# li-kunyi/CUT3R-SLAM

Measured on AMD Instinct MI355X. Metric: frames/sec (ViT pointmap + covisibility-graph tracking step) on 640x480, higher is better.
Workload: dtype f16

## Files before the change

### cut3r_slam_amd/_lib.py

```python
from __future__ import annotations

import ctypes as C
import os

_HERE = os.path.dirname(os.path.abspath(__file__))
LIB_PATH = os.path.join(_HERE, "libcut3r_hip.so")

c_void_p, c_int, c_float, c_ll = C.c_void_p, C.c_int, C.c_float, C.c_longlong


class GemmDesc(C.Structure):
    _fields_ = [
        ("A", c_void_p), ("B", c_void_p), ("C", c_void_p), ("bias", c_void_p), ("res1", c_void_p), ("res2", c_void_p),
        ("M", c_int), ("N", c_int), ("K", c_int), ("lda", c_int), ("ldb", c_int), ("ldc", c_int), ("ldr1", c_int),
        ("ldr2", c_int),
        ("act", c_int), ("out_f16", c_int), ("res1_f16", c_int), ("res2_f16", c_int),
        ("batch", c_int),
        ("strideA", c_ll), ("strideB", c_ll), ("strideC", c_ll), ("strideBias", c_ll), ("strideR1", c_ll),
        ("strideR2", c_ll),
        ("conv_k", c_int), ("H", c_int), ("W", c_int), ("Cin", c_int), ("conv_stride", c_int), ("Ho", c_int),
        ("Wo", c_int), ("relu_in", c_int),
        ("shuf", c_int), ("shuf_cout", c_int), ("shuf_Hin", c_int), ("shuf_Win", c_int),
        ("tile", c_int), ("stages", c_int),
        ("rope_pos", c_void_p), ("rope_table", c_void_p), ("rope_cols", c_int), ("rope_pmin", c_int), ("rope_npos", c_int),
# ... 21 lines not shown
    "cut3r_layernorm_tokens": [c_void_p, c_int, c_void_p, c_void_p, c_float, c_int, c_int, c_int, c_void_p, c_ll, c_void_p, c_ll, c_void_p,
                               c_ll, c_void_p, c_ll, c_void_p],
    "cut3r_gemm_f16": [C.POINTER(GemmDesc), c_void_p],
    "cut3r_gemm_tile_for": [C.POINTER(GemmDesc)],
    "cut3r_gemm_f16_pair": [C.POINTER(GemmDesc), C.POINTER(GemmDesc), c_void_p],
    "cut3r_gemm_kernel_for": [C.POINTER(GemmDesc)],
    "cut3r_gemm_pair_kernel_for": [C.POINTER(GemmDesc), C.POINTER(GemmDesc)],
    "cut3r_gemm_kernel_count": [],
    "cut3r_rope2d_table": [c_void_p, c_int, c_int, c_int, c_float, c_float, c_void_p],
    "cut3r_gemv_f16w": [c_void_p, c_int, c_void_p, c_int, c_void_p, c_void_p, c_int, c_int, c_int, c_int, c_int,
                        c_void_p, c_int, c_int, c_void_p],
    "cut3r_attention_variant": [c_int],
    "cut3r_attention_kernel_for": [c_int, c_int, c_int, c_int],
    "cut3r_attention_f16": [c_void_p, c_void_p, c_void_p, c_void_p, c_int, c_int, c_int, c_int, c_int,
                            c_ll, c_ll, c_ll, c_ll, c_ll, c_ll, c_ll, c_ll, c_float, c_void_p],
    "cut3r_attention_one_key_f16": [c_void_p, c_void_p, c_int, c_int, c_int, c_int, c_ll, c_ll, c_ll, c_ll, c_void_p],
    "cut3r_im2col_patch": [c_void_p, c_int, c_int, c_int, c_int, c_int, c_int, c_void_p, c_void_p],
    "cut3r_cast_f32_f16": [c_void_p, c_int, c_void_p, c_int, c_int, c_int, c_void_p],
    "cut3r_colmean": [c_void_p, c_int, c_int, c_int, c_void_p, c_void_p],
    "cut3r_colmean_batched": [c_void_p, c_int, c_ll, c_int, c_int, c_int, c_void_p, c_ll, c_void_p],
    "cut3r_upsample2x_nhwc": [c_void_p, c_void_p, c_int, c_int, c_int, c_int, c_void_p],
    "cut3r_dpt_final": [c_void_p, c_int, c_int, c_void_p, c_void_p, c_int, c_void_p, c_void_p, c_void_p],
    "cut3r_conv3x3_dpt_final": [C.POINTER(GemmDesc), c_void_p, c_void_p, c_int, c_void_p, c_ll, c_void_p, c_ll, c_void_p],
    "cut3r_postprocess_pts": [c_void_p, c_int, c_int, c_int, c_void_p, c_void_p, c_void_p],
    "cut3r_postprocess_pose": [c_void_p, c_int, c_void_p, c_void_p],
    "cut3r_patch_overlap": [c_void_p, c_void_p, c_int, c_int, c_float, c_void_p, c_void_p, c_void_p],
    "cut3r_patch_overlap_chain": [c_void_p, c_void_p, c_int, c_int, c_int, c_float, C.c_double, c_void_p, c_void_p, c_void_p, c_void_p,
                                  c_void_p, c_void_p],
    "cut3r_overlap_fwd": [c_void_p, c_int, C.POINTER(c_float), c_float, c_void_p, c_int, c_float, c_float, c_float, c_float,
                          c_int, c_int, c_int, c_void_p, c_void_p],
# ... 181 lines not shown
```

### cut3r_slam_amd/csrc/attention.hip

```cpp
#include <atomic>
#include <cmath>
#include <cstdlib>
#include <type_traits>
#include "common.h"
#include "../../include/cut3r_hip.h"

namespace {

typedef __fp16 fp16x4_t __attribute__((ext_vector_type(4)));

DEVINL void halves(float x, float& lo, float& hi) {
    const auto r = __builtin_amdgcn_permlane32_swap(__float_as_uint(x), __float_as_uint(x), false, false);
    lo = __uint_as_float(r[0]);
    hi = __uint_as_float(r[1]);
}

struct AttnArgs {
    const h16* q; const h16* k; const h16* v; h16* o;
    int Nq, Nk;
    long long q_sb, q_sn, k_sb, k_sn, v_sb, v_sn, o_sb, o_sn;
    float scale_log2;
};

template <int D, int NW>
// ... 217 lines not shown
DEVINL unsigned lds_addr(const void* p) {
    return (unsigned)(unsigned long long)(__attribute__((address_space(3))) const void*)p;
}

template <int N>
DEVINL void wait_vm() { asm volatile("s_waitcnt vmcnt(%0)" ::"n"(N) : "memory"); }
template <int P, int MAXT>
DEVINL void wait_tiles_ahead(int tiles_ahead) {
    if constexpr (MAXT == 0) wait_vm<0>();
    else {
        if (tiles_ahead >= MAXT) wait_vm<P * MAXT>();
        else wait_tiles_ahead<P, MAXT - 1>(tiles_ahead);
    }
}

template <int D, int QB, int NST, int NW>
__global__ __launch_bounds__(64 * NW, (QB == 1 ? 2 : 1)) void attn_pipe_kernel(const AttnArgs a, const int nblk, const int HB, const int H) {
    constexpr int KT = 64;
    constexpr int PPW = 8 / NW;
    constexpr int AHEAD = NST - 4;
    constexpr int DQ = D / 16;
    constexpr int DP = (D + 31) / 32;
    constexpr int CH = D / 8;
    constexpr int VOFF = KT * 128;
    constexpr int STAGE = 2 * KT * 128;
    static_assert(D % 16 == 0 && D <= 64 && NST >= 4 && (NW == 4 || NW == 8), "head dims 16..64; the ring holds tiles j-1 .. j+2 and NST-4 more in flight");
    __shared__ __attribute__((aligned(1024))) unsigned char smem[NST * STAGE];

    const int tid = threadIdx.x, lane = tid & 63;
    const int wave = __builtin_amdgcn_readfirstlane(tid >> 6);
    const int r = lane & 31, hh = lane >> 5;
    const int L = blockIdx.x;
    const int xb = (L >> 3) % nblk;
    const int bh = ((L >> 3) / nblk) * 8 + (L & 7);
    if (bh >= HB) return;
    const int h = bh % H, b = bh / H;
    const int q0 = xb * (32 * NW * QB) + wave * (32 * QB);
    const h16* qp = a.q + (size_t)b * a.q_sb + (size_t)h * D;
    const h16* kp = a.k + (size_t)b * a.k_sb + (size_t)h * D;
    const h16* vp = a.v + (size_t)b * a.v_sb + (size_t)h * D;
    const bool active = q0 < a.Nq;
    const int extra = (a.Nk > KT && (a.Nk % KT) == 1) ? 1 : 0;
    const int ntiles = (a.Nk - extra + KT - 1) / KT;

    if (CH < 8) {
        for (int i = tid; i < NST * STAGE / 16; i += 64 * NW) *reinterpret_cast<f32x4*>(smem + i * 16) = f32x4{0.f, 0.f, 0.f, 0.f};
        asm volatile("s_waitcnt lgkmcnt(0)" ::: "memory");
        asm volatile("s_barrier" ::: "memory");
    }

    auto lane_src = [&](int c, int row_limit, unsigned& ko, unsigned& vo, bool& kval, bool& vval) {
        const int row = (wave * PPW + c) * 8 + (lane >> 3), slot = lane & 7;
        const int kc = slot ^ ((row >> 1) & 7), vc = slot ^ (((row >> 1) & 1) << 2);
        const int rr = min(row, row_limit);
        ko = (unsigned)rr * (unsigned)(a.k_sn * 2) + kc * 16;
        vo = (unsigned)rr * (unsigned)(a.v_sn * 2) + vc * 16;
        kval = kc < CH;
        vval = vc < CH;
    };
// ... 32 lines not shown
            asm volatile("s_barrier" ::: "memory");
            issue(j + NST - 2);
        }
        asm volatile("s_waitcnt vmcnt(0)" ::: "memory");
        return;
    }

    half8_t qf[QB][DQ];
    f32x16 ot[QB][DP];
    float m_run[QB], l_run[QB];
#pragma unroll
    for (int qb = 0; qb < QB; qb++) {
        int qr = q0 + qb * 32 + r;
        if (qr > a.Nq - 1) qr = a.Nq - 1;
        const h16* qrow = qp + (size_t)qr * a.q_sn;
#pragma unroll
        for (int s = 0; s < DQ; s++) qf[qb][s] = *reinterpret_cast<const half8_t*>(qrow + 16 * s + 8 * hh);
#pragma unroll
        for (int d = 0; d < DP; d++)
#pragma unroll
            for (int i = 0; i < 16; i++) ot[qb][d][i] = 0.f;
        m_run[qb] = -INFINITY;
        l_run[qb] = 0.f;
        if (extra) {
            float dot = 0.f;
#pragma unroll
            for (int s = 0; s < DQ; s++) {
                const half8_t k0 = *reinterpret_cast<const half8_t*>(kp + 16 * s + 8 * hh);
#pragma unroll
                for (int j = 0; j < 8; j++) dot = fmaf((float)qf[qb][s][j], (float)k0[j], dot);
            }
            { float d0, d1; halves(dot, d0, d1); dot = d0 + d1; }
// ... 159 lines not shown
            if (__any(gflag)) {
#pragma unroll
                for (int qb = 0; qb < QB; qb++)
#pragma unroll
                    for (int d = 0; d < DP; d++)
#pragma unroll
                        for (int i = 0; i < 16; i++) ot[qb][d][i] *= alpha[qb];
            }
        }
    };
    using T0 = std::integral_constant<int, 0>;
    using T1 = std::integral_constant<int, 1>;
    using Y = std::true_type;
    using N = std::false_type;

#pragma unroll
    for (int t = 0; t < NST - 3; t++) issue(t);
    {
        wait_tiles_ahead<2 * PPW, AHEAD>(ntiles - 1);
        asm volatile("s_barrier" ::: "memory");
        issue(NST - 3);
        {
            half8_t kf[2][DQ];
#pragma unroll
            for (int kt2 = 0; kt2 < 2; kt2++)
#pragma unroll
                for (int s = 0; s < DQ; s++) kf[kt2][s] = *reinterpret_cast<const half8_t*>(smem + kt2 * 32 * 128 + koff[s]);
#pragma unroll
            for (int kt2 = 0; kt2 < 2; kt2++)
#pragma unroll
                for (int qb = 0; qb < QB; qb++) {
#pragma unroll
// ... 46 lines not shown
        }
    }
}

std::atomic<int> g_attn_variant{[] { const char* e = getenv("CUT3R_ATTN_PIPE"); return e ? atoi(e) : 1; }()};

int attn_instance(int B, int H, int Nq, int D) {
    static const long long nw4_min = [] { const char* e = getenv("CUT3R_ATTN_NW4_MIN"); return e ? atoll(e) : 384LL; }();
    if (D != 16 && D != 32 && D != 48 && D != 64 && D != 128) return 0;
    if ((D == 48 || D == 64) && g_attn_variant.load(std::memory_order_relaxed) != 0) return 104;
    const long long blocks128 = (long long)B * H * ((Nq + 127) / 128);
    return (blocks128 >= nw4_min || D >= 128) ? 4 : 2;
}

template <int D>
int launch_attn(const AttnArgs& a, int B, int H, hipStream_t s) {
    const int inst = attn_instance(B, H, a.Nq, D);
    if constexpr (D == 48 || D == 64) {
        if (inst == 104) {
            const int nblk = (a.Nq + 127) / 128, HB = H * B;
            dim3 grid((unsigned)(((HB + 7) / 8) * 8 * nblk));
            hipLaunchKernelGGL((attn_pipe_kernel<D, 1, 4, 4>), grid, dim3(256), 0, s, a, nblk, HB, H);
            return cut3r_check_launch();
        }
    }
    if (inst == 4) {
        dim3 grid((a.Nq + 127) / 128, H, B);
        hipLaunchKernelGGL((attn_kernel<D, 4>), grid, dim3(256), 0, s, a);
    } else if (inst == 2) {
        dim3 grid((a.Nq + 63) / 64, H, B);
        hipLaunchKernelGGL((attn_kernel<D, 2>), grid, dim3(128), 0, s, a);
    } else {
        return CUT3R_ERR_ARG;
    }
    return cut3r_check_launch();
}

__global__ __launch_bounds__(256) void attn_one_key_kernel(const h16* __restrict__ v, h16* __restrict__ o, int Nq, int hd8, long long v_sb,
                                                           long long o_sb, long long o_sn, long long total) {
    const long long i = (long long)blockIdx.x * 256 + threadIdx.x;
// ... 20 lines not shown
    hipLaunchKernelGGL(attn_one_key_kernel, dim3((unsigned)((total + 255) / 256)), dim3(256), 0, (hipStream_t)stream, (const h16*)v,
                       (h16*)out, Nq, (int)(hd / 8), v_sb, o_sb, o_sn, total);
    return cut3r_check_launch();
}

extern "C" int cut3r_attention_variant(int v) {
    if (v < 0) return g_attn_variant.load(std::memory_order_relaxed);
    return g_attn_variant.exchange(v ? 1 : 0, std::memory_order_relaxed);
}

extern "C" int cut3r_attention_kernel_for(int B, int H, int Nq, int D) {
    if (B <= 0 || H <= 0 || Nq <= 0) return 0;
    return attn_instance(B, H, Nq, D);
}

extern "C" int cut3r_attention_f16(const void* q, const void* k, const void* v, void* out, int B, int H, int Nq, int Nk, int D,
                                   long long q_sb, long long q_sn, long long k_sb, long long k_sn, long long v_sb, long long v_sn,
                                   long long o_sb, long long o_sn, float scale, void* stream) {
    if (!q || !k || !v || !out || B <= 0 || H <= 0 || Nq <= 0 || Nk <= 0) return CUT3R_ERR_ARG;
    if (((uintptr_t)q | (uintptr_t)k | (uintptr_t)v) & 15) return CUT3R_ERR_ARG;
    if ((uintptr_t)out & 7) return CUT3R_ERR_ARG;
    if ((q_sn | k_sn | v_sn | q_sb | k_sb | v_sb) & 7) return CUT3R_ERR_ARG;
    if ((o_sn | o_sb) & 3) return CUT3R_ERR_ARG;
    if (!(scale > 0.f) || !std::isfinite(scale)) return CUT3R_ERR_ARG;
    AttnArgs a;
    a.q = (const h16*)q; a.k = (const h16*)k; a.v = (const h16*)v; a.o = (h16*)out;
    a.Nq = Nq; a.Nk = Nk;
    a.q_sb = q_sb; a.q_sn = q_sn; a.k_sb = k_sb; a.k_sn = k_sn; a.v_sb = v_sb; a.v_sn = v_sn; a.o_sb = o_sb; a.o_sn = o_sn;
    a.scale_log2 = scale * 1.44269504088896340736f;
    hipStream_t s = (hipStream_t)stream;
    switch (D) {
        case 16: return launch_attn<16>(a, B, H, s);
        case 32: return launch_attn<32>(a, B, H, s);
        case 48: return launch_attn<48>(a, B, H, s);
        case 64: return launch_attn<64>(a, B, H, s);
        case 128: return launch_attn<128>(a, B, H, s);
        default: return CUT3R_ERR_ARG;
    }
}
```

### cut3r_slam_amd/model.py

```python
from __future__ import annotations

import contextlib
import gc
import math
import os
import re
from dataclasses import dataclass, field
from typing import Dict, List, NamedTuple, Optional

import torch

from . import ops
from .config import Cut3rConfig, production_config, state_dict_schema

F16, F32 = torch.float16, torch.float32


def _env_flag(name: str, default: bool) -> bool:
    return os.environ.get(name, "1" if default else "0") != "0"


def _env_int(name: str, default: int) -> int:
    return int(os.environ.get(name, str(default)))

# ... 27 lines not shown
    st: Optional[torch.Tensor] = None


@dataclass
class _Block:
    p: str
    tag: str
    x: _Stream
    y: _Stream
    out: _Stream
    xpos: Optional[torch.Tensor]
    ypos: Optional[torch.Tensor]
    heads: int
    B: int
    pre_ln: bool = False
    C: int = field(init=False)
    Nx: int = field(init=False)
    Ny: int = field(init=False)
    D: int = field(init=False)
    fold_x: bool = field(init=False, default=False)
    fold_y: bool = field(init=False, default=False)
    fold_o: bool = field(init=False, default=False)
    emit: Optional[tuple] = field(init=False, default=None)
    ln16: Optional[torch.Tensor] = field(init=False, default=None)
    y16: Optional[torch.Tensor] = field(init=False, default=None)
    qkv: Optional[torch.Tensor] = field(init=False, default=None)
    attn: Optional[torch.Tensor] = field(init=False, default=None)
    q: Optional[torch.Tensor] = field(init=False, default=None)
    kv: Optional[torch.Tensor] = field(init=False, default=None)
    cattn: Optional[torch.Tensor] = field(init=False, default=None)
# ... 17 lines not shown
            if tuple(state_dict[k].shape) != tuple(shp):
                raise ValueError(f"{k}: shape {tuple(state_dict[k].shape)} != schema {tuple(shp)}")
        self._buf: Dict[tuple, torch.Tensor] = {}
        self._graphs: Dict[tuple, tuple] = {}
        self.use_graphs = _env_flag("CUT3R_GRAPHS", True)
        self.dual_stream = _env_flag("CUT3R_DUAL_STREAM", True)
        self.dual_ln = _env_flag("CUT3R_DUAL_LN", True)
        self.pair_gemm = _env_flag("CUT3R_PAIR_GEMM", False)
        self.pair_rows = _env_int("CUT3R_PAIR_ROWS", 0)
        self.fused_rope = _env_int("CUT3R_FUSED_ROPE", 1)
        self.rope48_rows = _env_int("CUT3R_ROPE48_ROWS", 0)
        self.head_overlap = _env_flag("CUT3R_HEAD_OVERLAP", True)
        self.dpt_fuse = _env_flag("CUT3R_DPT_FUSE", True)
        self.head_chunk = max(1, _env_int("CUT3R_HEAD_CHUNK", 28))
        self.one_key = _env_flag("CUT3R_ONE_KEY", True)
        self.ln_fold = _env_int("CUT3R_LN_FOLD", 1)
        self._head_stream = None
        self._side = None
        self._head_side = None
        self._enc_last = None
        self._enc_events: Dict[int, torch.cuda.Event] = {}
        self._prep(state_dict)

    @classmethod
    def from_state_dict(cls, cfg, sd, device="cuda:0", **kw):
        return cls(cfg, sd, device, **kw)

    @classmethod
    def from_pretrained(cls, path: str, config: Optional[Cut3rConfig] = None, device="cuda:0", **kw):
        import argparse
# ... 68 lines not shown
        ln("enc_norm")
        lin("decoder_embed"); lin("decoder_embed_state")
        for i in range(cfg.dec_depth):
            dec_block(f"dec_blocks.{i}"); dec_block(f"dec_blocks_state.{i}")
        ln("dec_norm"); ln("dec_norm_state")
        lin("pose_retriever.proj_q")
        for i in range(2):
            dec_block(f"pose_retriever.write_blocks.{i}", False); dec_block(f"pose_retriever.read_blocks.{i}", False)
        self.pose_token = f32("pose_token").reshape(1, -1)
        self.masked_token = f32("pose_retriever.masked_token").reshape(1, -1)
        self.mem0 = f32("pose_retriever.mem").reshape(cfg.local_mem_size, -1)
        self.register_tokens16 = sd["register_tokens.weight"].to(device=dev, dtype=F16).contiguous()
        w = cfg.state_width
        i = torch.arange(cfg.state_size)
        self.state_pos = torch.stack([i // w, i % w], -1)[None].to(dev).contiguous()
        for hd in {cfg.enc_embed_dim // cfg.enc_num_heads, cfg.dec_embed_dim // cfg.dec_num_heads, cfg.dec_embed_dim // cfg.state_dec_num_heads}:
            if hd % 16 == 0:
                ops.rope_table(dev, cfg.rope_freq, 1.0, hd)
        h = "downstream_head"
        lin(h + ".pose_head.mlp.fc1"); lin(h + ".pose_head.mlp.fc2")
        if cfg.head_type == "dpt":
            self._prep_dpt(sd, h + ".dpt_self", 4)
            if not self.minimal:
                self._prep_dpt(sd, h + ".dpt_cross", 4)
                if cfg.rgb_head:
                    self._prep_dpt(sd, h + ".dpt_rgb", 3)
        else:
            lin(h + ".proj.fc1"); lin(h + ".proj.fc2")
            if not self.minimal:
                lin(h + ".cross_proj.fc1"); lin(h + ".cross_proj.fc2")
# ... 207 lines not shown
    def encode_image(self, view):
        img = view["img"]
        if not img.is_cuda:
            img = img.to(self.device)
        B = img.shape[0]
        im_shape = view.get("true_shape", torch.tensor(img.shape[-2:])[None].repeat(B, 1))
        img = img.to(F32) if img.dtype != torch.uint8 else img
        if self.use_graphs:
            with self._encoder_turn():
                feat, _, pos = self._graphed("enc", self._encode, img.contiguous())
                feat = feat.clone()
        else:
            feat, _, pos = self._encode(img)
        return feat, pos, im_shape

    def _block(self, p, tag, x, y, out, xpos, ypos, heads, B=1, fresh=False, pre_ln=False):
        s = _Block(p, tag, x, y, out, xpos, ypos, heads, B, pre_ln)
        C, Nx, Ny, D = s.C, s.Nx, s.Ny, s.D
        can = lambda t, n, name: bool(t.x16 is not None and n > 1 and self._folded(p + name))
        s.fold_x = fresh and can(x, Nx, ".attn.qkv")
        s.fold_y = fresh and can(y, Ny, ".cross_attn.projkv")
        s.fold_o = can(out, Nx, ".mlp.fc1")
        s.emit = (out.st, out.x16) if s.fold_o else None
        s.ln16 = self.buf(tag + ".ln16", (B * Nx, C), F16)
        s.y16 = self.buf(tag + ".y16", (B * Ny, C), F16)
        s.qkv = self.buf(tag + ".qkv", (B * Nx, 3 * C), F16)
        s.attn = self.buf(tag + ".attn", (B, Nx, heads, D), F16)
        s.q = self.buf(tag + ".q", (B, Nx, heads, D), F16)
        s.kv = self.buf(tag + ".kv", (B * Ny, 2 * C), F16)
        s.cattn = self.buf(tag + ".cattn", (B, Nx, heads, D), F16)
        s.mlp_h = self.buf(tag + ".mlp_h", (B * Nx, self.w[p + ".mlp.fc1"].npad), F16)
        return s
# ... 13 lines not shown
            todo = [s for s in blocks if need(s)]
            if fork and len(todo) == 2:
                cur = torch.cuda.current_stream()
                self._side.wait_stream(cur)
                with torch.cuda.stream(self._side):
                    fn(todo[0])
                fn(todo[1])
                cur.wait_stream(self._side)
            else:
                for s in todo:
                    fn(s)

        rows = lambda t: t.view(-1, t.shape[-2] * t.shape[-1])
        skx, sky = (lambda s: s.Nx == 1), (lambda s: s.Ny == 1)
        one_x, one_y = (lambda s: self.one_key and s.Nx == 1), (lambda s: self.one_key and s.Ny == 1)
        each(lambda s: self._ln(s.x.x, s.p + ".norm1", out16=s.ln16), lambda s: not (s.fold_x or s.pre_ln))
        self._project([dict(x16=s.x.x16 if s.fold_x else s.ln16, name=s.p + ".attn.qkv", out=s.qkv, skinny=skx(s),
                            rope=(s.xpos, 2 * s.C, s.D) if fuse_x(s) else None, ln=s.x.st if s.fold_x else None)
                       if not one_x(s) else
                       dict(x16=s.ln16, name=s.p + ".attn.qkv", out=rows(s.attn), skinny=True, cols=(2 * s.C, 3 * s.C)) for s in blocks])

        def self_attn(s):
            v5 = s.qkv.view(s.B, s.Nx, 3, s.heads, s.D)
            q, k, v = v5[:, :, 0], v5[:, :, 1], v5[:, :, 2]
            if s.xpos is not None and not fuse_x(s):
                ops.rope_2d_pair(q, s.xpos, k, s.xpos, self.cfg.rope_freq, 1.0)
            ops.attention(q, k, v, s.attn, s.D ** -0.5)
        each(self_attn, lambda s: not one_x(s))
        self._project([dict(x16=rows(s.attn), name=s.p + ".attn.proj", out=s.out.x, res1=s.x.x, skinny=skx(s), emit=s.emit) for s in blocks])
        each(lambda s: self._ln(s.out.x, s.p + ".norm2", out16=s.ln16), lambda s: not (s.fold_o or one_y(s)))
        self._project([dict(x16=s.out.x16 if s.fold_o else s.ln16, name=s.p + ".cross_attn.projq", out=rows(s.q), skinny=skx(s),
                            rope=(s.xpos, s.C, s.D) if fuse_x(s) else None, ln=s.out.st if s.fold_o else None) for s in blocks if not one_y(s)])
        rope_q = lambda s: s.xpos is not None and not fuse_x(s) and not one_y(s)
        rope_k = lambda s: s.ypos is not None and not fuse_y(s) and not one_y(s)
        rope_qk = lambda s: self.one_key and rope_q(s) and rope_k(s)
        norm_y = lambda s: not (s.fold_y or s.pre_ln)

        def q_rope_and_norm_y(s):
            if rope_q(s) and not rope_qk(s):
                self._rope(s.q, s.xpos)
            if norm_y(s):
                self._ln(s.y.x, s.p + ".norm_y", out16=s.y16)
        each(q_rope_and_norm_y, lambda s: (rope_q(s) and not rope_qk(s)) or norm_y(s))
        self._project([dict(x16=s.y.x16 if s.fold_y else s.y16, name=s.p + ".cross_attn.projkv", out=s.kv, skinny=sky(s),
                            rope=(s.ypos, s.C, s.D) if fuse_y(s) else None, ln=s.y.st if s.fold_y else None) for s in blocks])

        def cross_attn(s):
            kv4 = s.kv.view(s.B, s.Ny, 2, s.heads, s.D)
            k, v = kv4[:, :, 0], kv4[:, :, 1]
            if one_y(s):
                return ops.attention_one_key(v, s.cattn)
            if rope_qk(s):
                ops.rope_2d_pair(s.q, s.xpos, k, s.ypos, self.cfg.rope_freq, 1.0)
            elif s.ypos is not None and not fuse_y(s):
                self._rope(k, s.ypos)
            ops.attention(s.q, k, v, s.cattn, s.D ** -0.5)
        each(cross_attn)
        self._project([dict(x16=rows(s.cattn), name=s.p + ".cross_attn.proj", out=s.out.x, res1=s.out.x, skinny=skx(s), emit=s.emit) for s in blocks])
        each(lambda s: self._ln(s.out.x, s.p + ".norm3", out16=s.ln16), lambda s: not s.fold_o)
        self._project([dict(x16=s.out.x16 if s.fold_o else s.ln16, name=s.p + ".mlp.fc1", out=s.mlp_h, skinny=skx(s),
                            ln=s.out.st if s.fold_o else None) for s in blocks], act=1)
        self._project([dict(x16=s.mlp_h, name=s.p + ".mlp.fc2", out=s.out.x, res1=s.out.x, skinny=skx(s), emit=s.emit) for s in blocks])

    def _dual_norms(self, l, a, s_a):
        pi, ps = f"dec_blocks.{l}", f"dec_blocks_state.{l}"
        Ci = a.shape[1]
        ops.layernorm_dual(a, *self.w[pi + ".norm1"], self.buf("deci.ln16", (a.shape[0], Ci), F16),
                           *self.w[ps + ".norm_y"], self.buf("decs.y16", (a.shape[0], Ci), F16), self.cfg.ln_eps)
        ops.layernorm_dual(s_a, *self.w[ps + ".norm1"], self.buf("decs.ln16", (s_a.shape[0], Ci), F16),
                           *self.w[pi + ".norm_y"], self.buf("deci.y16", (s_a.shape[0], Ci), F16), self.cfg.ln_eps)
# ... 142 lines not shown

    def _decode(self, feat, feat16, H, W, return_taps=False):
        cfg = self.cfg
        P, E, D, Ld = cfg.patch_size, cfg.enc_embed_dim, cfg.dec_embed_dim, cfg.dec_depth
        Wn, V, N, _ = feat.shape
        nh, nw = H // P, W // P
        S = cfg.state_size
        dev = self.device
        if feat16 is None:
            feat16 = self.buf("win.feat16", (Wn, V, N, E), F16)
            ops.cast_f16(feat.reshape(Wn * V * N, E), feat16.view(Wn * V * N, E))
        y, xx = torch.meshgrid(torch.arange(nh, device=dev), torch.arange(nw, device=dev), indexing="ij")
        pos1 = torch.stack([y.reshape(-1), xx.reshape(-1)], -1)[None]
        pos_img = torch.cat([-torch.ones(1, 1, 2, dtype=torch.int64, device=dev), pos1], dim=1).expand(Wn, -1, -1).contiguous()
        pos_state = self.state_pos.expand(Wn, -1, -1).contiguous()
        taps = {"enc_feat": feat[0]} if return_taps else None

        small = self._pair_carries(Wn * max(N + 1, S))
        pair = self.pair_gemm or small
        fold = self.ln_fold and D % 64 == 0 and self._folded("dec_blocks.0.attn.qkv") and (small or not pair)

        def stream(name, rows):
            x = self.buf(name, (rows, D), F32)
            return _Stream(x, *self._xs(name, x)) if fold else _Stream(x)
        st = [stream("dec.state0", Wn * S), stream("dec.state1", Wn * S)]
        im = [stream("dec.img0", Wn * (N + 1)), stream("dec.img1", Wn * (N + 1))]
        s0 = self.buf("dec.s0", (S, D), F32)
        self._linear(self.register_tokens16, "decoder_embed_state", s0)
        st[0].x.view(Wn, S, D).copy_(s0[None].expand(Wn, -1, -1))
        msz = self.mem0.shape[0]
# ... 32 lines not shown
            a, b = im[0], im[1]
            a3 = a.x.view(Wn, N + 1, D)
            if i == 0:
                a3[:, 0] = self.pose_token
            else:
                a3[:, 0] = self._mem_inquire(g16, mem[cm], Wn)
            ops.linear_batched(feat16[:, i], w_de, a3[:, 1:], b_de)
            s_a, s_b = st[cs], st[cs ^ 1]
            dead_tail = (i == V - 1) and not return_taps
            fresh = False
            for l in range(Ld):
                last = dead_tail and l == Ld - 1
                pre = bool(not last and self.dual_ln and D in (768, 1024, 1536) and not (fold and fresh))
                if pre:
                    self._dual_norms(l, a.x, s_a.x)
                image = self._block(f"dec_blocks.{l}", "deci", a, s_a, b, pos_img, pos_state, cfg.dec_num_heads, Wn, fresh, pre)
                state = None if last else self._block(f"dec_blocks_state.{l}", "decs", s_a, a, s_b, pos_state, pos_img, cfg.state_dec_num_heads,
                                                      Wn, fresh, pre)
                if last:
                    self._dec_layer([image])
                elif pair:
                    self._dec_layer([state, image], fork)
                elif fork:
                    cur = torch.cuda.current_stream()
                    self._side.wait_stream(cur)
                    with torch.cuda.stream(self._side):
                        self._dec_layer([state])
                    self._dec_layer([image])
                    cur.wait_stream(self._side)
                else:
                    self._dec_layer([state])
                    self._dec_layer([image])
                s_a, s_b = s_b, s_a
# ... 191 lines not shown
```

### cut3r_slam_amd/ops.py

```python
from __future__ import annotations

import ctypes as C
import os
from typing import Optional

import torch

from . import _lib, views
from ._lib import GemmDesc, check

F16, F32 = torch.float16, torch.float32


def _stream():
    return C.c_void_p(torch.cuda.current_stream().cuda_stream)


def _p(t: Optional[torch.Tensor]):
    return C.c_void_p(t.data_ptr()) if t is not None else C.c_void_p(0)


def _req(cond, msg):
    if not cond:
        raise ValueError(msg)
# ... 339 lines not shown
    _cuda(q, k, v, out)
    B, Nq, H, D = q.shape
    Nk = k.shape[1]
    for t in (q, k, v, out):
        _req(t.dtype == F16 and t.dim() == 4 and t.stride(3) == 1 and t.stride(2) == D, "attention operands: fp16 (B,N,H,D) views")
    _req(k.shape == (B, Nk, H, D) and v.shape == (B, Nk, H, D) and out.shape == (B, Nq, H, D), "attention shapes")
    _req(D in (16, 32, 48, 64, 128), f"unsupported head dim {D}")
    _req(0.0 < float(scale) < float("inf"), f"attention scale must be finite and > 0, got {scale}")
    lib = _lib.load()
    check(lib.cut3r_attention_f16(_p(q), _p(k), _p(v), _p(out), B, H, Nq, Nk, D, q.stride(0), q.stride(1), k.stride(0),
                                  k.stride(1), v.stride(0), v.stride(1), out.stride(0), out.stride(1), float(scale),
                                  _stream()), f"cut3r_attention_f16 B={B} H={H} Nq={Nq} Nk={Nk} D={D}")
    return out


def attention_one_key(v, out):
    _cuda(v, out)
    for t in (v, out):
        _req(t.dtype == F16 and t.dim() == 4 and t.stride(3) == 1 and t.stride(2) == t.shape[3], "attention operands: fp16 (B,N,H,D) views")
    B, Nq, H, D = out.shape
    _req(v.shape == (B, 1, H, D), "attention_one_key: v [B,1,H,D]")
    _req(D % 8 == 0 and D <= 256, f"unsupported head dim {D}")
    _aligned(16, v=v, out=out)
    lib = _lib.load()
    check(lib.cut3r_attention_one_key_f16(_p(v), _p(out), B, H, Nq, D, v.stride(0), v.stride(1), out.stride(0), out.stride(1), _stream()),
          f"cut3r_attention_one_key_f16 B={B} H={H} Nq={Nq} D={D}")
    return out


def im2col_patch(img, P, out):
# ... 1170 lines not shown
```

### include/cut3r_hip.h

```cpp
#ifndef CUT3R_HIP_H
#define CUT3R_HIP_H
#include <stdint.h>
#ifdef __cplusplus
extern "C" {
#endif

int cut3r_abi_version(void);

int cut3r_rope2d(void* tokens, int dtype, const int64_t* positions, int B, int N, int H, int D,
                 long long sB, long long sN, long long sH, float base, float fwd, void* stream);
int cut3r_rope2d_qk(void* q, void* k, int dtype, const int64_t* positions, int B, int N, int H, int D, long long q_sB,
                    long long q_sN, long long k_sB, long long k_sN, float base, float fwd, void* stream);

int cut3r_rope2d_tab(void* t0, const int64_t* pos0, long long ntok0, long long stride0, void* t1, const int64_t* pos1, long long ntok1,
                     long long stride1, int H, int D, const float* table, int pmin, int npos, float base, float fwd, void* stream);

int cut3r_layernorm(const float* x, int ldx, const float* gamma, const float* beta, float eps, int M, int C,
                    void* y16, int ld16, float* y32, int ld32, const float* mod_scale, const float* mod_shift,
                    void* stream);
int cut3r_layernorm_dual(const float* x, int ldx, const float* g1, const float* b1, void* y1, int ld1, const float* g2,
                         const float* b2, void* y2, int ld2, float eps, int M, int C, void* stream);
int cut3r_layernorm_tokens(const float* x, int ldx, const float* gamma, const float* beta, float eps, int Wn, int N, int C,
                           float* pose32, long long pose32_gs, void* pose16, long long pose16_gs, void* tok16, long long tok16_gs,
                           float* tok32, long long tok32_gs, void* stream);
// ... 37 lines not shown
int cut3r_gemm_pair_kernel_for(const cut3r_gemm_desc* d0, const cut3r_gemm_desc* d1);
int cut3r_gemm_kernel_count(void);

int cut3r_gemv_f16w(const float* X, int ldx, const void* W, int ldw, const float* bias, float* Y, int ldy,
                    int M, int N, int K, int act, const float* res, int ldr, int silu_in, void* stream);

int cut3r_attention_f16(const void* q, const void* k, const void* v, void* out, int B, int H, int Nq, int Nk, int D,
                        long long q_sb, long long q_sn, long long k_sb, long long k_sn, long long v_sb, long long v_sn,
                        long long o_sb, long long o_sn, float scale, void* stream);

int cut3r_attention_one_key_f16(const void* v, void* out, int B, int H, int Nq, int D, long long v_sb, long long v_sn, long long o_sb,
                                long long o_sn, void* stream);

int cut3r_attention_variant(int v);
int cut3r_attention_kernel_for(int B, int H, int Nq, int D);

int cut3r_im2col_patch(const void* img, int u8, int B, int C, int H, int W, int P, void* out, void* stream);
int cut3r_cast_f32_f16(const float* x, int ldx, void* y, int ldy, int M, int C, void* stream);
int cut3r_colmean(const float* x, int ldx, int M, int C, float* y, void* stream);
int cut3r_colmean_batched(const float* x, int B, long long stride_x, int ldx, int M, int C, float* y, long long stride_y, void* stream);

int cut3r_upsample2x_nhwc(const void* in, void* out, int B, int H, int W, int C, void* stream);
int cut3r_dpt_final(const void* in, int P, int Cin, const float* w, const float* b, int mode, float* pts, float* conf,
                    void* stream);
int cut3r_conv3x3_dpt_final(const cut3r_gemm_desc* d, const float* w, const float* b, int mode, float* pts, long long pts_view_stride,
                            float* conf, long long conf_view_stride, void* stream);
int cut3r_postprocess_pts(const float* raw, int P, int nch, int pos_z, float* pts, float* conf, void* stream);
int cut3r_postprocess_pose(const float* raw, int B, float* out, void* stream);

int cut3r_patch_overlap(const float* feat0, const float* feat1, int N, int C, float thr, void* ws, int32_t* count,
// ... 284 lines not shown
```

Measured before the change: 5842.

## Fuse query RoPE into the pipelined attention kernel's Q load

Adds a ROPEQ variant of the pipelined attention kernel that reads raw Q, looks up cos/sin from the RoPE table using the per-token positions, and rotates Q in registers before the QK product. The first K/V tile DMAs are issued before the rotation so the table loads overlap the prefetch. The decoder self- and cross-attention paths use it when the positions fall inside the table and the pipe kernel is selected, leaving only K to be rotated separately. This removes a separate RoPE pass over Q and its global read/write, in exchange for extra register pressure and table loads inside the attention kernel.

```diff
diff --git a/cut3r_slam_amd/_lib.py b/cut3r_slam_amd/_lib.py
--- a/cut3r_slam_amd/_lib.py
+++ b/cut3r_slam_amd/_lib.py
@@ -59,6 +59,9 @@
     "cut3r_attention_kernel_for": [c_int, c_int, c_int, c_int],
     "cut3r_attention_f16": [c_void_p, c_void_p, c_void_p, c_void_p, c_int, c_int, c_int, c_int, c_int,
                             c_ll, c_ll, c_ll, c_ll, c_ll, c_ll, c_ll, c_ll, c_float, c_void_p],
+    "cut3r_attention_rope_q_ok": [c_int, c_int, c_int, c_int],
+    "cut3r_attention_rope_q_f16": [c_void_p, c_void_p, c_void_p, c_void_p, c_int, c_int, c_int, c_int, c_int,
+                                   c_ll, c_ll, c_ll, c_ll, c_ll, c_ll, c_ll, c_ll, c_float, c_void_p, c_void_p, c_int, c_int, c_void_p],
     "cut3r_attention_one_key_f16": [c_void_p, c_void_p, c_int, c_int, c_int, c_int, c_ll, c_ll, c_ll, c_ll, c_void_p],
     "cut3r_im2col_patch": [c_void_p, c_int, c_int, c_int, c_int, c_int, c_int, c_void_p, c_void_p],
     "cut3r_cast_f32_f16": [c_void_p, c_int, c_void_p, c_int, c_int, c_int, c_void_p],
diff --git a/cut3r_slam_amd/csrc/attention.hip b/cut3r_slam_amd/csrc/attention.hip
--- a/cut3r_slam_amd/csrc/attention.hip
+++ b/cut3r_slam_amd/csrc/attention.hip
@@ -255,8 +255,15 @@
     }
 }
 
-template <int D, int QB, int NST, int NW>
-__global__ __launch_bounds__(64 * NW, (QB == 1 ? 2 : 1)) void attn_pipe_kernel(const AttnArgs a, const int nblk, const int HB, const int H) {
+struct RopeQArgs {
+    const int64_t* pos;
+    const float* table;
+    int pmin, npos;
+};
+
+template <int D, int QB, int NST, int NW, bool ROPEQ = false>
+__global__ __launch_bounds__(64 * NW, (QB == 1 ? 2 : 1)) void attn_pipe_kernel(const AttnArgs a, const int nblk, const int HB, const int H,
+                                                                              const RopeQArgs rq) {
     constexpr int KT = 64;
     constexpr int PPW = 8 / NW;
     constexpr int AHEAD = NST - 4;
@@ -284,6 +291,16 @@
     const int extra = (a.Nk > KT && (a.Nk % KT) == 1) ? 1 : 0;
     const int ntiles = (a.Nk - extra + KT - 1) / KT;
 
+    long long qpos[QB][2] = {};
+    if constexpr (ROPEQ) {
+#pragma unroll
+        for (int qb = 0; qb < QB; qb++) {
+            const int qr = min(q0 + qb * 32 + r, a.Nq - 1);
+            const int64_t* pp = rq.pos + ((size_t)b * a.Nq + qr) * 2;
+            qpos[qb][0] = pp[0];
+            qpos[qb][1] = pp[1];
+        }
+    }
     if (CH < 8) {
         for (int i = tid; i < NST * STAGE / 16; i += 64 * NW) *reinterpret_cast<f32x4*>(smem + i * 16) = f32x4{0.f, 0.f, 0.f, 0.f};
         asm volatile("s_waitcnt lgkmcnt(0)" ::: "memory");
@@ -346,8 +363,60 @@
         int qr = q0 + qb * 32 + r;
         if (qr > a.Nq - 1) qr = a.Nq - 1;
         const h16* qrow = qp + (size_t)qr * a.q_sn;
-#pragma unroll
-        for (int s = 0; s < DQ; s++) qf[qb][s] = *reinterpret_cast<const half8_t*>(qrow + 16 * s + 8 * hh);
+        if constexpr (!ROPEQ) {
+#pragma unroll
+            for (int s = 0; s < DQ; s++) qf[qb][s] = *reinterpret_cast<const half8_t*>(qrow + 16 * s + 8 * hh);
+        } else {
+            constexpr int Q = D / 4;
+            long long pi[2];
+#pragma unroll
+            for (int X = 0; X < 2; X++) {
+                const long long p = qpos[qb][X] - rq.pmin;
+                pi[X] = p < 0 ? 0 : (p > rq.npos - 1 ? rq.npos - 1 : p);
+            }
+            half8_t own[DQ];
+            half4_t par[DQ][2];
+            f32x4 c4[DQ][2], s4[DQ][2];
+            unsigned sgn[DQ][2];
+#pragma unroll
+            for (int s = 0; s < DQ; s++) {
+                const int c0 = 16 * s + 8 * hh;
+                own[s] = *reinterpret_cast<const half8_t*>(qrow + c0);
+                const float* tc = rq.table + (((hh ? 16 * s + 8 : 16 * s) / (2 * Q)) ? pi[1] : pi[0]) * Q;
+                const float* ts = tc + (long long)rq.npos * Q;
+#pragma unroll
+                for (int g = 0; g < 2; g++) {
+                    const int w = hh ? (16 * s + 8 + 4 * g) % (2 * Q) : (16 * s + 4 * g) % (2 * Q);
+                    const bool isv = w >= Q;
+                    const int f0 = isv ? w - Q : w;
+                    par[s][g] = *reinterpret_cast<const half4_t*>(qrow + c0 + 4 * g + (isv ? -Q : Q));
+                    c4[s][g] = *reinterpret_cast<const f32x4*>(tc + f0);
+                    s4[s][g] = *reinterpret_cast<const f32x4*>(ts + f0);
+                    sgn[s][g] = isv ? 0u : 0x80000000u;
+                }
+            }
+            static_assert(QB == 1, "the early request belongs to the one query block of the workgroup");
+#pragma unroll
+            for (int t = 0; t < NST - 3; t++) issue(t);
+#pragma unroll
+            for (int s = 0; s < DQ; s++)
+#pragma unroll
+                for (int g = 0; g < 2; g++) asm volatile("" ::"v"(own[s]), "v"(par[s][g]), "v"(c4[s][g]), "v"(s4[s][g]));
+#pragma unroll
+            for (int s = 0; s < DQ; s++) {
+                half8_t rot;
+#pragma unroll
+                for (int g = 0; g < 2; g++)
+#pragma unroll
+                    for (int j = 0; j < 4; j++) {
+                        const float af = (float)own[s][4 * g + j], pf = (float)par[s][g][j];
+                        float t = pf * s4[s][g][j];
+                        asm volatile("" : "+v"(t));
+                        rot[4 * g + j] = (h16)rope_rot(af, c4[s][g][j], __uint_as_float(__float_as_uint(t) ^ sgn[s][g]));
+                    }
+                qf[qb][s] = rot;
+            }
+        }
 #pragma unroll
         for (int d = 0; d < DP; d++)
 #pragma unroll
@@ -537,8 +606,10 @@
     using Y = std::true_type;
     using N = std::false_type;
 
-#pragma unroll
-    for (int t = 0; t < NST - 3; t++) issue(t);
+    if constexpr (!ROPEQ) {
+#pragma unroll
+        for (int t = 0; t < NST - 3; t++) issue(t);
+    }
     {
         wait_tiles_ahead<2 * PPW, AHEAD>(ntiles - 1);
         asm volatile("s_barrier" ::: "memory");
@@ -615,16 +686,18 @@
 }
 
 template <int D>
-int launch_attn(const AttnArgs& a, int B, int H, hipStream_t s) {
+int launch_attn(const AttnArgs& a, int B, int H, hipStream_t s, const RopeQArgs* rq = nullptr) {
     const int inst = attn_instance(B, H, a.Nq, D);
     if constexpr (D == 48 || D == 64) {
         if (inst == 104) {
             const int nblk = (a.Nq + 127) / 128, HB = H * B;
             dim3 grid((unsigned)(((HB + 7) / 8) * 8 * nblk));
-            hipLaunchKernelGGL((attn_pipe_kernel<D, 1, 4, 4>), grid, dim3(256), 0, s, a, nblk, HB, H);
+            if (rq) hipLaunchKernelGGL((attn_pipe_kernel<D, 1, 4, 4, true>), grid, dim3(256), 0, s, a, nblk, HB, H, *rq);
+            else hipLaunchKernelGGL((attn_pipe_kernel<D, 1, 4, 4>), grid, dim3(256), 0, s, a, nblk, HB, H, RopeQArgs{});
             return cut3r_check_launch();
         }
     }
+    if (rq) return CUT3R_ERR_ARG;
     if (inst == 4) {
         dim3 grid((a.Nq + 127) / 128, H, B);
         hipLaunchKernelGGL((attn_kernel<D, 4>), grid, dim3(256), 0, s, a);
@@ -675,9 +748,14 @@
     return attn_instance(B, H, Nq, D);
 }
 
-extern "C" int cut3r_attention_f16(const void* q, const void* k, const void* v, void* out, int B, int H, int Nq, int Nk, int D,
-                                   long long q_sb, long long q_sn, long long k_sb, long long k_sn, long long v_sb, long long v_sn,
-                                   long long o_sb, long long o_sn, float scale, void* stream) {
+extern "C" int cut3r_attention_rope_q_ok(int B, int H, int Nq, int D) {
+    if (B <= 0 || H <= 0 || Nq <= 0 || (D != 48 && D != 64)) return 0;
+    return attn_instance(B, H, Nq, D) == 104 ? 1 : 0;
+}
+
+static int attention_f16(const void* q, const void* k, const void* v, void* out, int B, int H, int Nq, int Nk, int D, long long q_sb,
+                         long long q_sn, long long k_sb, long long k_sn, long long v_sb, long long v_sn, long long o_sb, long long o_sn,
+                         float scale, const RopeQArgs* rq, void* stream) {
     if (!q || !k || !v || !out || B <= 0 || H <= 0 || Nq <= 0 || Nk <= 0) return CUT3R_ERR_ARG;
     if (((uintptr_t)q | (uintptr_t)k | (uintptr_t)v) & 15) return CUT3R_ERR_ARG;
     if ((uintptr_t)out & 7) return CUT3R_ERR_ARG;
@@ -690,12 +768,30 @@
     a.q_sb = q_sb; a.q_sn = q_sn; a.k_sb = k_sb; a.k_sn = k_sn; a.v_sb = v_sb; a.v_sn = v_sn; a.o_sb = o_sb; a.o_sn = o_sn;
     a.scale_log2 = scale * 1.44269504088896340736f;
     hipStream_t s = (hipStream_t)stream;
+    if (rq) {
+        if (!cut3r_attention_rope_q_ok(B, H, Nq, D)) return CUT3R_ERR_ARG;
+        if (!rq->pos || !rq->table || rq->npos <= 0 || ((uintptr_t)rq->pos & 7) || ((uintptr_t)rq->table & 15)) return CUT3R_ERR_ARG;
+    }
     switch (D) {
         case 16: return launch_attn<16>(a, B, H, s);
         case 32: return launch_attn<32>(a, B, H, s);
-        case 48: return launch_attn<48>(a, B, H, s);
-        case 64: return launch_attn<64>(a, B, H, s);
+        case 48: return launch_attn<48>(a, B, H, s, rq);
+        case 64: return launch_attn<64>(a, B, H, s, rq);
         case 128: return launch_attn<128>(a, B, H, s);
         default: return CUT3R_ERR_ARG;
     }
 }
+
+extern "C" int cut3r_attention_f16(const void* q, const void* k, const void* v, void* out, int B, int H, int Nq, int Nk, int D,
+                                   long long q_sb, long long q_sn, long long k_sb, long long k_sn, long long v_sb, long long v_sn,
+                                   long long o_sb, long long o_sn, float scale, void* stream) {
+    return attention_f16(q, k, v, out, B, H, Nq, Nk, D, q_sb, q_sn, k_sb, k_sn, v_sb, v_sn, o_sb, o_sn, scale, nullptr, stream);
+}
+
+extern "C" int cut3r_attention_rope_q_f16(const void* q, const void* k, const void* v, void* out, int B, int H, int Nq, int Nk, int D,
+                                          long long q_sb, long long q_sn, long long k_sb, long long k_sn, long long v_sb, long long v_sn,
+                                          long long o_sb, long long o_sn, float scale, const int64_t* q_pos, const float* table, int pmin,
+                                          int npos, void* stream) {
+    const RopeQArgs rq{q_pos, table, pmin, npos};
+    return attention_f16(q, k, v, out, B, H, Nq, Nk, D, q_sb, q_sn, k_sb, k_sn, v_sb, v_sn, o_sb, o_sn, scale, &rq, stream);
+}
diff --git a/cut3r_slam_amd/model.py b/cut3r_slam_amd/model.py
--- a/cut3r_slam_amd/model.py
+++ b/cut3r_slam_amd/model.py
@@ -65,6 +65,7 @@
     heads: int
     B: int
     pre_ln: bool = False
+    xpos_in_table: bool = False
     C: int = field(init=False)
     Nx: int = field(init=False)
     Ny: int = field(init=False)
@@ -112,6 +113,7 @@
         self.dpt_fuse = _env_flag("CUT3R_DPT_FUSE", True)
         self.head_chunk = max(1, _env_int("CUT3R_HEAD_CHUNK", 28))
         self.one_key = _env_flag("CUT3R_ONE_KEY", True)
+        self.rope_q_attn = _env_flag("CUT3R_ROPE_Q_ATTN", True)
         self.ln_fold = _env_int("CUT3R_LN_FOLD", 1)
         self._head_stream = None
         self._side = None
@@ -210,6 +212,7 @@
         w = cfg.state_width
         i = torch.arange(cfg.state_size)
         self.state_pos = torch.stack([i // w, i % w], -1)[None].to(dev).contiguous()
+        self._state_pos_in_table = ops.rope_positions_in_table(self.state_pos)
         for hd in {cfg.enc_embed_dim // cfg.enc_num_heads, cfg.dec_embed_dim // cfg.dec_num_heads, cfg.dec_embed_dim // cfg.state_dec_num_heads}:
             if hd % 16 == 0:
                 ops.rope_table(dev, cfg.rope_freq, 1.0, hd)
@@ -447,8 +450,8 @@
             feat, _, pos = self._encode(img)
         return feat, pos, im_shape
 
-    def _block(self, p, tag, x, y, out, xpos, ypos, heads, B=1, fresh=False, pre_ln=False):
-        s = _Block(p, tag, x, y, out, xpos, ypos, heads, B, pre_ln)
+    def _block(self, p, tag, x, y, out, xpos, ypos, heads, B=1, fresh=False, pre_ln=False, xpos_in_table=False):
+        s = _Block(p, tag, x, y, out, xpos, ypos, heads, B, pre_ln, xpos_in_table)
         C, Nx, Ny, D = s.C, s.Nx, s.Ny, s.D
         can = lambda t, n, name: bool(t.x16 is not None and n > 1 and self._folded(p + name))
         s.fold_x = fresh and can(x, Nx, ".attn.qkv")
@@ -492,6 +495,8 @@
         rows = lambda t: t.view(-1, t.shape[-2] * t.shape[-1])
         skx, sky = (lambda s: s.Nx == 1), (lambda s: s.Ny == 1)
         one_x, one_y = (lambda s: self.one_key and s.Nx == 1), (lambda s: self.one_key and s.Ny == 1)
+        rope_q_attn = lambda s: bool(self.rope_q_attn and s.xpos is not None and s.xpos_in_table and not fuse_x(s) and not one_x(s)
+                                     and not one_y(s) and ops.attention_rope_q_ok(s.B, s.heads, s.Nx, s.D))
         each(lambda s: self._ln(s.x.x, s.p + ".norm1", out16=s.ln16), lambda s: not (s.fold_x or s.pre_ln))
         self._project([dict(x16=s.x.x16 if s.fold_x else s.ln16, name=s.p + ".attn.qkv", out=s.qkv, skinny=skx(s),
                             rope=(s.xpos, 2 * s.C, s.D) if fuse_x(s) else None, ln=s.x.st if s.fold_x else None)
@@ -501,6 +506,9 @@
         def self_attn(s):
             v5 = s.qkv.view(s.B, s.Nx, 3, s.heads, s.D)
             q, k, v = v5[:, :, 0], v5[:, :, 1], v5[:, :, 2]
+            if rope_q_attn(s):
+                self._rope(k, s.xpos)
+                return ops.attention_rope_q(q, s.xpos, k, v, s.attn, s.D ** -0.5, self.cfg.rope_freq)
             if s.xpos is not None and not fuse_x(s):
                 ops.rope_2d_pair(q, s.xpos, k, s.xpos, self.cfg.rope_freq, 1.0)
             ops.attention(q, k, v, s.attn, s.D ** -0.5)
@@ -509,7 +517,7 @@
         each(lambda s: self._ln(s.out.x, s.p + ".norm2", out16=s.ln16), lambda s: not (s.fold_o or one_y(s)))
         self._project([dict(x16=s.out.x16 if s.fold_o else s.ln16, name=s.p + ".cross_attn.projq", out=rows(s.q), skinny=skx(s),
                             rope=(s.xpos, s.C, s.D) if fuse_x(s) else None, ln=s.out.st if s.fold_o else None) for s in blocks if not one_y(s)])
-        rope_q = lambda s: s.xpos is not None and not fuse_x(s) and not one_y(s)
+        rope_q = lambda s: s.xpos is not None and not fuse_x(s) and not one_y(s) and not rope_q_attn(s)
         rope_k = lambda s: s.ypos is not None and not fuse_y(s) and not one_y(s)
         rope_qk = lambda s: self.one_key and rope_q(s) and rope_k(s)
         norm_y = lambda s: not (s.fold_y or s.pre_ln)
@@ -532,6 +540,8 @@
                 ops.rope_2d_pair(s.q, s.xpos, k, s.ypos, self.cfg.rope_freq, 1.0)
             elif s.ypos is not None and not fuse_y(s):
                 self._rope(k, s.ypos)
+            if rope_q_attn(s):
+                return ops.attention_rope_q(s.q, s.xpos, k, v, s.cattn, s.D ** -0.5, self.cfg.rope_freq)
             ops.attention(s.q, k, v, s.cattn, s.D ** -0.5)
         each(cross_attn)
         self._project([dict(x16=rows(s.cattn), name=s.p + ".cross_attn.proj", out=s.out.x, res1=s.out.x, skinny=skx(s), emit=s.emit) for s in blocks])
@@ -704,6 +714,7 @@
         pos1 = torch.stack([y.reshape(-1), xx.reshape(-1)], -1)[None]
         pos_img = torch.cat([-torch.ones(1, 1, 2, dtype=torch.int64, device=dev), pos1], dim=1).expand(Wn, -1, -1).contiguous()
         pos_state = self.state_pos.expand(Wn, -1, -1).contiguous()
+        img_pos_in_table = ops.ROPE_PMIN <= -1 and max(nh, nw) <= ops.ROPE_PMIN + ops.ROPE_NPOS
         taps = {"enc_feat": feat[0]} if return_taps else None
 
         small = self._pair_carries(Wn * max(N + 1, S))
@@ -766,9 +777,9 @@
                 pre = bool(not last and self.dual_ln and D in (768, 1024, 1536) and not (fold and fresh))
                 if pre:
                     self._dual_norms(l, a.x, s_a.x)
-                image = self._block(f"dec_blocks.{l}", "deci", a, s_a, b, pos_img, pos_state, cfg.dec_num_heads, Wn, fresh, pre)
+                image = self._block(f"dec_blocks.{l}", "deci", a, s_a, b, pos_img, pos_state, cfg.dec_num_heads, Wn, fresh, pre, img_pos_in_table)
                 state = None if last else self._block(f"dec_blocks_state.{l}", "decs", s_a, a, s_b, pos_state, pos_img, cfg.state_dec_num_heads,
-                                                      Wn, fresh, pre)
+                                                      Wn, fresh, pre, self._state_pos_in_table)
                 if last:
                     self._dec_layer([image])
                 elif pair:
diff --git a/cut3r_slam_amd/ops.py b/cut3r_slam_amd/ops.py
--- a/cut3r_slam_amd/ops.py
+++ b/cut3r_slam_amd/ops.py
@@ -377,6 +377,37 @@
     return out
 
 
+def attention_rope_q_ok(B, H, Nq, D):
+    return bool(_lib.load().cut3r_attention_rope_q_ok(int(B), int(H), int(Nq), int(D)))
+
+
+def rope_positions_in_table(pos):
+    lo, hi = (int(x) for x in torch.aminmax(pos)) if pos.numel() else (ROPE_PMIN, ROPE_PMIN)
+    return ROPE_PMIN <= lo and hi < ROPE_PMIN + ROPE_NPOS
+
+
+def attention_rope_q(q, q_pos, k, v, out, scale, base, check_positions=False):
+    _cuda(q, k, v, out, q_pos)
+    B, Nq, H, D = q.shape
+    Nk = k.shape[1]
+    for t in (q, k, v, out):
+        _req(t.dtype == F16 and t.dim() == 4 and t.stride(3) == 1 and t.stride(2) == D, "attention operands: fp16 (B,N,H,D) views")
+    _req(k.shape == (B, Nk, H, D) and v.shape == (B, Nk, H, D) and out.shape == (B, Nq, H, D), "attention shapes")
+    _req(D in (48, 64), f"attention_rope_q: heads of 48 or 64, got {D}")
+    _req(0.0 < float(scale) < float("inf"), f"attention scale must be finite and > 0, got {scale}")
+    _req(q_pos.shape == (B, Nq, 2) and q_pos.dtype == torch.int64 and q_pos.is_contiguous(), "positions must be contiguous int64 [B,Nq,2]")
+    lib = _lib.load()
+    _req(lib.cut3r_attention_rope_q_ok(B, H, Nq, D) == 1, "attention_rope_q: the pipelined attention kernel is switched off (CUT3R_ATTN_PIPE)")
+    if check_positions:
+        _req(rope_positions_in_table(q_pos), f"attention_rope_q: positions outside the table [{ROPE_PMIN}, {ROPE_PMIN + ROPE_NPOS})")
+    tab = rope_table(q.device, base, 1.0, D)
+    check(lib.cut3r_attention_rope_q_f16(_p(q), _p(k), _p(v), _p(out), B, H, Nq, Nk, D, q.stride(0), q.stride(1), k.stride(0),
+                                         k.stride(1), v.stride(0), v.stride(1), out.stride(0), out.stride(1), float(scale), _p(q_pos),
+                                         _p(tab), ROPE_PMIN, ROPE_NPOS, _stream()),
+          f"cut3r_attention_rope_q_f16 B={B} H={H} Nq={Nq} Nk={Nk} D={D}")
+    return out
+
+
 def attention_one_key(v, out):
     _cuda(v, out)
     for t in (v, out):
diff --git a/include/cut3r_hip.h b/include/cut3r_hip.h
--- a/include/cut3r_hip.h
+++ b/include/cut3r_hip.h
@@ -75,6 +75,12 @@
 
 int cut3r_attention_variant(int v);
 int cut3r_attention_kernel_for(int B, int H, int Nq, int D);
+
+int cut3r_attention_rope_q_f16(const void* q, const void* k, const void* v, void* out, int B, int H, int Nq, int Nk, int D,
+                               long long q_sb, long long q_sn, long long k_sb, long long k_sn, long long v_sb, long long v_sn,
+                               long long o_sb, long long o_sn, float scale, const int64_t* q_pos, const float* table, int pmin, int npos,
+                               void* stream);
+int cut3r_attention_rope_q_ok(int B, int H, int Nq, int D);
 
 int cut3r_im2col_patch(const void* img, int u8, int B, int C, int H, int W, int P, void* out, void* stream);
 int cut3r_cast_f32_f16(const float* x, int ldx, void* y, int ldy, int M, int C, void* stream);
```

Measured after the change: 5857 (median of 5 runs). About the same (+0.3%).
